# Borda/pyImSegm

Measured on NVIDIA H100. Metric: megapixels/sec end-to-end SLIC+features+GC (pipe_color2d_slic_features_model_graphcut), higher is better.
Workload: dtype f64

## Files before the change

### pyimsegm_b200/csrc/common.cuh

```cuda
#pragma once
#include <cuda_runtime.h>
#include <stdint.h>
#include <stdio.h>
#include "../../include/imsegm_b200.h"

void isb_set_error(const char* fmt, ...);
extern long long g_isb_launches;

enum {
    ISB_PROF_PREPARE = 0, ISB_PROF_ASSIGN, ISB_PROF_UPDATE, ISB_PROF_FINALIZE, ISB_PROF_CONN, ISB_PROF_STATS, ISB_PROF_ADJ,
    ISB_PROF_ENERGY, ISB_PROF_GC, ISB_PROF_GATHER, ISB_PROF_GMM, ISB_PROF_LM, ISB_PROF_COUNT
};
int isb_prof_begin(int id, cudaStream_t st);
void isb_prof_end(int handle, cudaStream_t st);
struct ProfScope {
    int h; cudaStream_t st;
    ProfScope(int id, cudaStream_t s) : h(isb_prof_begin(id, s)), st(s) {}
    ~ProfScope() { if (h >= 0) isb_prof_end(h, st); }
};

#define ISB_CUDA_CHECK(call)                                                                      \
    do {                                                                                          \
        cudaError_t e__ = (call);                                                                 \
        if (e__ != cudaSuccess) {                                                                 \
            isb_set_error("%s:%d %s -> %s", __FILE__, __LINE__, #call, cudaGetErrorString(e__));  \
            return ISB_ERR_CUDA;                                                                  \
        }                                                                                         \
    } while (0)

#define ISB_LAUNCH_CHECK()                                                                        \
    do {                                                                                          \
        ++g_isb_launches;                                                                         \
        cudaError_t e__ = cudaGetLastError();                                                     \
        if (e__ != cudaSuccess) {                                                                 \
            isb_set_error("%s:%d kernel launch -> %s", __FILE__, __LINE__, cudaGetErrorString(e__)); \
            return ISB_ERR_CUDA;                                                                  \
        }                                                                                         \
    } while (0)

#define ISB_REQUIRE(cond, msg)                                          \
    do {                                                                \
        if (!(cond)) {                                                  \
            isb_set_error("%s:%d %s", __FILE__, __LINE__, msg);         \
            return ISB_ERR_ARG;                                         \
        }                                                               \
    } while (0)

static inline size_t isb_align(size_t x, size_t a = 256) { return (x + a - 1) / a * a; }

struct WsCarver {
    char* base;
    size_t off, cap;
    WsCarver(void* p, size_t bytes) : base((char*)p), off(0), cap(bytes) {}
    template <typename T> T* take(size_t n)
    {
        size_t o = isb_align(off);
        off = o + n * sizeof(T);
        return (T*)(base + o);
    }
    bool ok() const { return off <= cap; }
};

__device__ __forceinline__ double load_as_f64(const void* p, int dtype, size_t i)
{
    switch (dtype) {
        case ISB_U8: return (double)((const unsigned char*)p)[i];
        case ISB_U16: return (double)((const unsigned short*)p)[i];
        case ISB_F32: return (double)((const float*)p)[i];
        default: return ((const double*)p)[i];
    }
}

__device__ __forceinline__ float load_as_f32(const void* p, int dtype, size_t i)
{
    switch (dtype) {
        case ISB_U8: return (float)((const unsigned char*)p)[i];
        case ISB_U16: return (float)((const unsigned short*)p)[i];
        case ISB_F32: return ((const float*)p)[i];
        default: return (float)((const double*)p)[i];
    }
}

__device__ __forceinline__ unsigned long long f64_ordered(double d)
{
    unsigned long long u = (unsigned long long)__double_as_longlong(d);
    return (u & 0x8000000000000000ull) ? ~u : (u | 0x8000000000000000ull);
}
__device__ __forceinline__ double f64_unordered(unsigned long long u)
{
    u = (u & 0x8000000000000000ull) ? (u & 0x7FFFFFFFFFFFFFFFull) : ~u;
    return __longlong_as_double((long long)u);
}

__device__ __forceinline__ int reflect_index(int i, int n)
{
    if ((unsigned)i < (unsigned)n) return i;
    if (n == 1) return 0;
    int p = 2 * n;
    i %= p;
    if (i < 0) i += p;
    return (i < n) ? i : (p - 1 - i);
}
```

### pyimsegm_b200/csrc/graph.cu

```cuda
#include "common.cuh"
#include "block_scan.cuh"
#include <cooperative_groups.h>
namespace cg = cooperative_groups;

namespace {


struct AdjWs {
    unsigned long long* table;
    int* ctr;
    int* deg;
    int* off;
    int* fill;
    int* tmp_a;
    int slots;
    size_t zeroed;
};

__device__ __forceinline__ unsigned hash64(unsigned long long k)
{
    k ^= k >> 33; k *= 0xff51afd7ed558ccdull; k ^= k >> 33; k *= 0xc4ceb9fe1a85ec53ull; k ^= k >> 33;
    return (unsigned)k;
}

__device__ __forceinline__ unsigned long long edge_key(int l0, int l1)
{
    return ((unsigned long long)(unsigned)max(l0, l1) << 32) | (unsigned)min(l0, l1);
}

__device__ void table_insert(const AdjWs& w, unsigned long long key)
{
    unsigned mask = (unsigned)w.slots - 1u;
    unsigned h = hash64(key) & mask;
    for (int probe = 0; probe < w.slots; ++probe) {
        unsigned long long cur = w.table[h];
        if (cur == key) return;
        if (cur == 0) {
            unsigned long long old = atomicCAS(&w.table[h], 0ull, key);
            if (old == 0) { atomicAdd(&w.deg[key >> 32], 1); atomicAdd(&w.ctr[0], 1); return; }
            if (old == key) return;
        }
        h = (h + 1) & mask;
    }
    atomicExch(&w.ctr[1], 1);
}

constexpr int CTA_SLOTS = 512, CTA_PROBES = 32;

__device__ void cta_set_clear(unsigned long long* s)
{
    for (int i = threadIdx.x; i < CTA_SLOTS; i += blockDim.x) s[i] = 0;
    __syncthreads();
}

__device__ void cta_set_insert(unsigned long long* s, const AdjWs& w, unsigned long long key)
{
    unsigned h = hash64(key) & (CTA_SLOTS - 1);
    for (int probe = 0; probe < CTA_PROBES; ++probe) {
        unsigned long long cur = s[h];
        if (cur == key) return;
        if (cur == 0) {
            cur = atomicCAS(&s[h], 0ull, key);
            if (cur == 0 || cur == key) return;
        }
        h = (h + 1) & (CTA_SLOTS - 1);
    }
    table_insert(w, key);
}

__device__ void cta_set_flush(const unsigned long long* s, const AdjWs& w)
{
    __syncthreads();
    for (int i = threadIdx.x; i < CTA_SLOTS; i += blockDim.x)
        if (s[i]) table_insert(w, s[i]);
}

constexpr int ETW = 64, ETR = 4, ETH = ETR * (256 / ETW);

__global__ void __launch_bounds__(256) k_edge_scan(const int* __restrict__ seg, int H, int W, AdjWs w)
{
    __shared__ unsigned long long s_set[CTA_SLOTS];
    cta_set_clear(s_set);
    const int x = blockIdx.x * ETW + (int)(threadIdx.x % ETW);
    const int y0 = blockIdx.y * ETH + (int)(threadIdx.x / ETW) * ETR, y1 = min(y0 + ETR, H);
    if (x < W && y0 < H) {
        unsigned long long last = 0;
        int l = seg[(size_t)y0 * W + x];
        for (int y = y0; y < y1; ++y) {
            const size_t p = (size_t)y * W + x;
            const int d = y + 1 < H ? seg[p + W] : l;
            if (x + 1 < W) {
                const int r = seg[p + 1];
                if (r != l && edge_key(l, r) != last) { last = edge_key(l, r); cta_set_insert(s_set, w, last); }
            }
            if (d != l && edge_key(l, d) != last) { last = edge_key(l, d); cta_set_insert(s_set, w, last); }
            l = d;
        }
    }
    cta_set_flush(s_set, w);
}

__global__ void __launch_bounds__(256) k_edge_scan3d(const int* __restrict__ seg, int D, int H, int W, AdjWs w)
{
    __shared__ unsigned long long s_set[CTA_SLOTS];
    cta_set_clear(s_set);
    const size_t p = (size_t)blockIdx.x * blockDim.x + threadIdx.x;
    if (p < (size_t)D * H * W) {
        const int x = (int)(p % W), y = (int)((p / W) % H), z = (int)(p / ((size_t)H * W));
        const int l = seg[p];
        if (x + 1 < W) { const int r = seg[p + 1]; if (r != l) cta_set_insert(s_set, w, edge_key(l, r)); }
        if (y + 1 < H) { const int d = seg[p + W]; if (d != l) cta_set_insert(s_set, w, edge_key(l, d)); }
        if (z + 1 < D) { const int b = seg[p + (size_t)H * W]; if (b != l) cta_set_insert(s_set, w, edge_key(l, b)); }
    }
    cta_set_flush(s_set, w);
}

__global__ void k_centroid3d_acc(const int* __restrict__ seg, int D, int H, int W, unsigned long long* acc)
{
    size_t p = (size_t)blockIdx.x * blockDim.x + threadIdx.x;
    if (p >= (size_t)D * H * W) return;
    const int x = (int)(p % W), y = (int)((p / W) % H), z = (int)(p / ((size_t)H * W));
    unsigned long long* a = acc + 4 * (size_t)seg[p];
    atomicAdd(a, 1ull); atomicAdd(a + 1, (unsigned long long)z); atomicAdd(a + 2, (unsigned long long)y); atomicAdd(a + 3, (unsigned long long)x);
}

__global__ void k_centroid3d_fin(int nb, const unsigned long long* acc, double* centres)
{
    const int k = blockIdx.x * blockDim.x + threadIdx.x;
    if (k >= nb) return;
    const double c = (double)acc[4 * (size_t)k];
    for (int d = 0; d < 3; ++d) centres[3 * (size_t)k + d] = c > 0 ? (double)acc[4 * (size_t)k + 1 + d] / c : -1.0;
}

__global__ void __launch_bounds__(1024) k_edge_offsets(int nb, AdjWs w, int cap, int* n_edges_out)
{
    const int total = cta_scan_chunks<1024, int>(nb, [&](int i) { return w.deg[i]; },
                                                 [&](int i, int off) { w.off[i] = off; w.fill[i] = 0; });
    if (threadIdx.x == 0) {
        w.off[nb] = total;
        *n_edges_out = (w.ctr[1] || total > cap) ? cap + 1 : total;
    }
}

__global__ void k_edge_fill(AdjWs w, int cap)
{
    int i = blockIdx.x * blockDim.x + threadIdx.x;
    if (i >= w.slots) return;
    unsigned long long key = w.table[i];
    if (key == 0) return;
    int b = (int)(key >> 32), a = (int)(key & 0xffffffffu);
    int pos = w.off[b] + atomicAdd(&w.fill[b], 1);
    if (pos < cap) w.tmp_a[pos] = a;
}

__global__ void k_edge_emit(int nb, AdjWs w, int cap, int* __restrict__ edges)
{
    int b = blockIdx.x * blockDim.x + threadIdx.x;
    if (b >= nb) return;
    int beg = w.off[b], end = w.off[b + 1];
    if (end > cap) return;
    for (int i = beg + 1; i < end; ++i) {
        int v = w.tmp_a[i], j = i - 1;
        while (j >= beg && w.tmp_a[j] > v) { w.tmp_a[j + 1] = w.tmp_a[j]; --j; }
        w.tmp_a[j + 1] = v;
    }
    for (int i = beg; i < end; ++i) { edges[2 * (size_t)i] = w.tmp_a[i]; edges[2 * (size_t)i + 1] = b; }
}

static int pow2_at_least(long long v) { int p = 1024; while (p < v) p <<= 1; return p; }

static size_t carve_adj(AdjWs& w, void* ws, size_t bytes, int nb, int cap)
{
    WsCarver c(ws, bytes);
    w.slots = pow2_at_least(2LL * cap);
    w.table = c.take<unsigned long long>((size_t)w.slots);
    w.ctr = c.take<int>(4);
    w.deg = c.take<int>(nb);
    w.zeroed = c.off;
    w.off = c.take<int>((size_t)nb + 1);
    w.fill = c.take<int>(nb);
    w.tmp_a = c.take<int>(cap);
    return isb_align(c.off);
}


__device__ double block_sum(double v, double* s_red)
{
#pragma unroll
    for (int o = 16; o > 0; o >>= 1) v += __shfl_xor_sync(0xffffffffu, v, o);
    __syncthreads();
    if ((threadIdx.x & 31) == 0) s_red[threadIdx.x >> 5] = v;
    __syncthreads();
    double t = 0;
    for (int i = 0; i < (int)(blockDim.x >> 5); ++i) t += s_red[i];
    return t;
}

__device__ double block_max(double v, double* s_red)
{
#pragma unroll
    for (int o = 16; o > 0; o >>= 1) v = fmax(v, __shfl_xor_sync(0xffffffffu, v, o));
    __syncthreads();
    if ((threadIdx.x & 31) == 0) s_red[threadIdx.x >> 5] = v;
    __syncthreads();
    double t = s_red[0];
    for (int i = 1; i < (int)(blockDim.x >> 5); ++i) t = fmax(t, s_red[i]);
    return t;
}

constexpr int ECL = 8;

__device__ double cluster_reduce(double v, bool is_max, double* s_red, double* s_x)
{
    const double t = is_max ? block_max(v, s_red) : block_sum(v, s_red);
    cg::cluster_group cl = cg::this_cluster();
    if (threadIdx.x == 0) *s_x = t;
    cl.sync();
    double tot = is_max ? -1.0 : 0.0;
    for (int r = 0; r < ECL; ++r) { const double pr = *cl.map_shared_rank(s_x, r); tot = is_max ? fmax(tot, pr) : tot + pr; }
    cl.sync();
    return tot;
}

__global__ void __cluster_dims__(ECL, 1, 1) __launch_bounds__(1024) k_gc_energies(const double* __restrict__ proba, int N_in, const int* n_nodes_dev, int K, const int* __restrict__ edges, int E_in,
                                                      const int* n_edges_dev, const double* __restrict__ centres,
                                                      const double* __restrict__ vfeat, int D, int metric, int spatial,
                                                      double edge_cost, const double* __restrict__ pairwise, double* unary,
                                                      double* edge_w, int* unary_i, int* edge_wi, int* smooth_i, double* sp)
{
    __shared__ double s_red[32];
    __shared__ double s_x;
    const int tid = blockIdx.x * blockDim.x + threadIdx.x, nth = gridDim.x * blockDim.x;
    const int E = n_edges_dev ? (*n_edges_dev > E_in ? 0 : *n_edges_dev) : E_in;
    const int N = n_nodes_dev ? min(*n_nodes_dev, N_in) : N_in;
    double umax = 0.0;
    for (int i = tid; i < N * K; i += nth) {
        double p = proba[i];
        if (p < 0.01) p = 0.01;
        if (p > 1.0 - 0.01) p = 1.0 - 0.01;
        double u = fabs(-log(p));
        unary[i] = u;
        umax = fmax(umax, fabs(u));
    }
    umax = cluster_reduce(umax, true, s_red, &s_x);
    double dsum = 0.0, ssum = 0.0;
    for (int e = tid; e < E; e += nth) {
        int a = edges[2 * e], b = edges[2 * e + 1];
        double dist = 0.0;
        if (metric != 0) {
            const double* va = vfeat + (size_t)a * D;
            const double* vb = vfeat + (size_t)b * D;
            for (int k = 0; k < D; ++k) {
                double df = va[k] - vb[k];
                if (metric == 1) dist = fmax(dist, df * df);
                else if (metric == 2) dist += fabs(df);
                else dist += df * df;
            }
            if (metric == 3) dist = sqrt(dist);
        }
        edge_w[e] = dist;
        dsum += dist;
        if (spatial == 3) {
            const double cz = centres[3 * a] - centres[3 * b], cy = centres[3 * a + 1] - centres[3 * b + 1];
            const double cx = centres[3 * a + 2] - centres[3 * b + 2];
            const double s = sqrt(cz * cz + cy * cy + cx * cx);
            sp[e] = s;
            ssum += s;
        } else if (spatial) {
            double cy = centres[2 * a] - centres[2 * b], cx = centres[2 * a + 1] - centres[2 * b + 1];
            double s = sqrt(cy * cy + cx * cx);
            sp[e] = s;
            ssum += s;
        }
    }
    dsum = cluster_reduce(dsum, false, s_red, &s_x);
    ssum = cluster_reduce(ssum, false, s_red, &s_x);
    const double dmean = E > 0 ? dsum / E : 0.0, smean = E > 0 ? ssum / E : 1.0;
    double vsum = 0.0;
    if (metric != 0)
        for (int e = tid; e < E; e += nth) { double t = edge_w[e] - dmean; vsum += t * t; }
    vsum = cluster_reduce(vsum, false, s_red, &s_x);
    const double sd = sqrt(E > 0 ? vsum / E : 0.0);
    const double denom = 2.0 * (sd * sd);
    double wmax = 0.0;
    for (int e = tid; e < E; e += nth) {
        double wv = metric != 0 ? exp(-edge_w[e] / denom) : 1.0;
        if (spatial) wv = wv / (sp[e] / smean);
        if (wv < 1e-3) wv = 1e-3;
        if (wv > 1e3) wv = 1e3;
        wv *= edge_cost;
        edge_w[e] = wv;
        wmax = fmax(wmax, fabs(wv));
    }
    wmax = cluster_reduce(wmax, true, s_red, &s_x);
    double pmax = pairwise[0];
    for (int i = 1; i < K * K; ++i) pmax = fmax(pmax, pairwise[i]);
    const double dwf = fmax(umax, wmax * pmax) + 1e-10;
    for (int i = tid; i < N * K; i += nth) unary_i[i] = (int)((unary[i] / dwf) * 100000.0);
    for (int e = tid; e < E; e += nth) { const double wv = edge_w[e]; edge_wi[e] = isnan(wv) ? 0 : (int)((wv / dwf) * 1000.0); }
    for (int i = tid; i < K * K; i += nth) smooth_i[i] = (int)(pairwise[i] * 100.0);
}


constexpr int GV = 4, GW = 32 * GV;

__global__ void __launch_bounds__(256) k_gather(const int* __restrict__ seg, long long n, long long n_vec, const int* __restrict__ lut_i,
                                                const double* __restrict__ lut_p, int K, int* __restrict__ out_i, double* __restrict__ out_p)
{
    __shared__ int s_lab[256 * GV];
    const long long p0 = ((long long)blockIdx.x * blockDim.x + threadIdx.x) * GV;
    if (p0 >= n) return;
    if (p0 < n_vec) {
        const int4 l = *reinterpret_cast<const int4*>(seg + p0);
        if (out_i) *reinterpret_cast<int4*>(out_i + p0) = make_int4(__ldg(lut_i + l.x), __ldg(lut_i + l.y), __ldg(lut_i + l.z), __ldg(lut_i + l.w));
        if (out_p) {
            const int lane = threadIdx.x & 31;
            *reinterpret_cast<int4*>(s_lab + threadIdx.x * GV) = l;
            __syncwarp();
            const int* lab = s_lab + (threadIdx.x - lane) * GV;
            double2* dst = reinterpret_cast<double2*>(out_p + (p0 - lane * GV) * K);
            int q = 2 * lane / K, k = 2 * lane % K;
            const int dq = 64 / K, dk = 64 % K;
#pragma unroll 2
            for (int i = lane; i < GW * K / 2; i += 32) {
                const double v0 = __ldg(lut_p + (size_t)lab[q] * K + k);
                const int q1 = k + 1 == K ? q + 1 : q, k1 = k + 1 == K ? 0 : k + 1;
                const double v1 = __ldg(lut_p + (size_t)lab[q1] * K + k1);
                dst[i] = make_double2(v0, v1);
                q += dq; k += dk;
                if (k >= K) { k -= K; ++q; }
            }
        }
        return;
    }
    for (long long p = p0; p < min(p0 + GV, n); ++p) {
        const int l = seg[p];
        if (out_i) out_i[p] = lut_i[l];
        if (out_p) {
            const double* src = lut_p + (size_t)l * K;
            double* dst = out_p + (size_t)p * K;
            for (int k = 0; k < K; ++k) dst[k] = src[k];
        }
    }
}

}

extern "C" size_t isb_adjacency_workspace_bytes(int nb, int cap)
{
    AdjWs w;
    return carve_adj(w, nullptr, 0, nb, cap);
}

extern "C" int isb_adjacency_edges(const int32_t* seg, int H, int W, int nb, int32_t* edges, int cap, int32_t* n_edges_out, void* ws,
                                   size_t ws_bytes, isb_stream_t stream)
{
    ISB_REQUIRE(seg && edges && n_edges_out && ws, "null pointer");
    ISB_REQUIRE(H > 0 && W > 0 && nb > 0 && cap > 0, "bad sizes");
    ISB_REQUIRE((H + ETH - 1) / ETH <= 65535, "label map taller than the scan grid (1 048 560 rows)");
    AdjWs w;
    size_t need = carve_adj(w, ws, ws_bytes, nb, cap);
    ISB_REQUIRE(need <= ws_bytes, "workspace too small");
    cudaStream_t st = (cudaStream_t)stream;
    ProfScope prof(ISB_PROF_ADJ, st);
    ISB_CUDA_CHECK(cudaMemsetAsync(w.table, 0, w.zeroed, st));
    k_edge_scan<<<dim3((W + ETW - 1) / ETW, (H + ETH - 1) / ETH), 256, 0, st>>>(seg, H, W, w);
    ISB_LAUNCH_CHECK();
    k_edge_offsets<<<1, 1024, 0, st>>>(nb, w, cap, n_edges_out);
    ISB_LAUNCH_CHECK();
    k_edge_fill<<<(w.slots + 255) / 256, 256, 0, st>>>(w, cap);
    ISB_LAUNCH_CHECK();
    k_edge_emit<<<(nb + 127) / 128, 128, 0, st>>>(nb, w, cap, edges);
    ISB_LAUNCH_CHECK();
    return ISB_OK;
}

extern "C" int isb_adjacency_edges_3d(const int32_t* seg, int D, int H, int W, int nb, int32_t* edges, int cap, int32_t* n_edges_out,
                                      void* ws, size_t ws_bytes, isb_stream_t stream)
{
    ISB_REQUIRE(seg && edges && n_edges_out && ws, "null pointer");
    ISB_REQUIRE(D > 0 && H > 0 && W > 0 && nb > 0 && cap > 0, "bad sizes");
    AdjWs w;
    size_t need = carve_adj(w, ws, ws_bytes, nb, cap);
    ISB_REQUIRE(need <= ws_bytes, "workspace too small");
    cudaStream_t st = (cudaStream_t)stream;
    ProfScope prof(ISB_PROF_ADJ, st);
    ISB_CUDA_CHECK(cudaMemsetAsync(w.table, 0, w.zeroed, st));
    size_t n = (size_t)D * H * W;
    k_edge_scan3d<<<(unsigned)((n + 255) / 256), 256, 0, st>>>(seg, D, H, W, w);
    ISB_LAUNCH_CHECK();
    k_edge_offsets<<<1, 1024, 0, st>>>(nb, w, cap, n_edges_out);
    ISB_LAUNCH_CHECK();
    k_edge_fill<<<(w.slots + 255) / 256, 256, 0, st>>>(w, cap);
    ISB_LAUNCH_CHECK();
    k_edge_emit<<<(nb + 127) / 128, 128, 0, st>>>(nb, w, cap, edges);
    ISB_LAUNCH_CHECK();
    return ISB_OK;
}

extern "C" int isb_centroids_3d(const int32_t* seg, int D, int H, int W, int nb, double* centres, void* ws, size_t ws_bytes, isb_stream_t stream)
{
    ISB_REQUIRE(seg && centres && ws, "null pointer");
    ISB_REQUIRE(D > 0 && H > 0 && W > 0 && nb > 0, "bad sizes");
    ISB_REQUIRE(ws_bytes >= sizeof(unsigned long long) * 4 * (size_t)nb, "workspace too small (4 * nb uint64)");
    cudaStream_t st = (cudaStream_t)stream;
    ISB_CUDA_CHECK(cudaMemsetAsync(ws, 0, sizeof(unsigned long long) * 4 * (size_t)nb, st));
    size_t n = (size_t)D * H * W;
    k_centroid3d_acc<<<(unsigned)((n + 255) / 256), 256, 0, st>>>(seg, D, H, W, (unsigned long long*)ws);
    ISB_LAUNCH_CHECK();
    k_centroid3d_fin<<<(nb + 255) / 256, 256, 0, st>>>(nb, (const unsigned long long*)ws, centres);
    ISB_LAUNCH_CHECK();
    return ISB_OK;
}

extern "C" size_t isb_gc_energies_workspace_bytes(int N, int K, int E) { return isb_align(sizeof(double) * (size_t)(E > 0 ? E : 1)); }

extern "C" int isb_gc_energies(const double* proba, int N, const int32_t* n_nodes_dev, int K, const int32_t* edges, int E, const int32_t* n_edges_dev,
                               const double* centres, int metric, int spatial, double edge_cost, const double* pairwise, double* unary,
                               double* edge_w, int32_t* unary_i, int32_t* edge_wi, int32_t* smooth_i, void* ws, size_t ws_bytes,
                               isb_stream_t stream)
{
    ISB_REQUIRE(proba && edges && pairwise && unary && edge_w && unary_i && edge_wi && smooth_i && ws, "null pointer");
    ISB_REQUIRE(N > 0 && K > 0 && E >= 0, "bad sizes");
    ISB_REQUIRE(metric >= 0 && metric <= 3, "metric must be 0..3");
    ISB_REQUIRE(spatial >= 0 && spatial <= 3, "spatial must be 0 (off), 1 or 2 (centres [N, 2]) or 3 (centres [N, 3])");
    ISB_REQUIRE(!spatial || centres, "centres are required for spatially normalised edge weights");
    ISB_REQUIRE(ws_bytes >= isb_gc_energies_workspace_bytes(N, K, E), "workspace too small");
    ProfScope prof(ISB_PROF_ENERGY, (cudaStream_t)stream);
    k_gc_energies<<<ECL, 1024, 0, (cudaStream_t)stream>>>(proba, N, n_nodes_dev, K, edges, E, n_edges_dev, centres, proba, K, metric, spatial, edge_cost,
                                                         pairwise, unary, edge_w, unary_i, edge_wi, smooth_i, (double*)ws);
    ISB_LAUNCH_CHECK();
    return ISB_OK;
}

__global__ void k_fill_i32(int* p, long long n, int v)
{
    long long i = (long long)blockIdx.x * blockDim.x + threadIdx.x;
    if (i < n) p[i] = v;
}

extern "C" int isb_fill_i32(int32_t* dst, long long n, int32_t value, isb_stream_t stream)
{
    ISB_REQUIRE(dst && n > 0, "bad arguments");
    k_fill_i32<<<(unsigned)((n + 255) / 256), 256, 0, (cudaStream_t)stream>>>(dst, n, value);
    ISB_LAUNCH_CHECK();
    return ISB_OK;
}

__global__ void k_combine(void* dst, const void* src, long long n, int op)
{
    long long i = (long long)blockIdx.x * blockDim.x + threadIdx.x;
    if (i >= n) return;
    if (op == 0) ((long long*)dst)[i] += ((const long long*)src)[i];
    else if (op == 1) { long long a = ((long long*)dst)[i], b = ((const long long*)src)[i]; ((long long*)dst)[i] = a > b ? a : b; }
    else if (op == 2 || op == 3) {
        const double a = ((double*)dst)[i], b = ((const double*)src)[i];
        ((double*)dst)[i] = (a != a || b != b) ? a + b : (op == 2 ? fmin(a, b) : fmax(a, b));
    }
    else ((double*)dst)[i] = ((double*)dst)[i] + ((const double*)src)[i];
}

extern "C" int isb_combine(void* dst, const void* src, long long n, int op, isb_stream_t stream)
{
    ISB_REQUIRE(dst && src && n > 0 && op >= 0 && op <= 4, "bad arguments");
    k_combine<<<(unsigned)((n + 255) / 256), 256, 0, (cudaStream_t)stream>>>(dst, src, n, op);
    ISB_LAUNCH_CHECK();
    return ISB_OK;
}

extern "C" int isb_gather(const int32_t* seg, long long npx, const int32_t* lut_i, const double* lut_p, int K, int32_t* out_i,
                          double* out_p, isb_stream_t stream)
{
    ISB_REQUIRE(seg && npx > 0, "bad arguments");
    ISB_REQUIRE((!out_i || lut_i) && (!out_p || (lut_p && K > 0)), "LUT missing for a requested output");
    ProfScope prof(ISB_PROF_GATHER, (cudaStream_t)stream);
    const bool aligned = (((uintptr_t)seg | (uintptr_t)out_i | (uintptr_t)out_p) & 15) == 0;
    const long long groups = (npx + GV - 1) / GV;
    k_gather<<<(unsigned)((groups + 255) / 256), 256, 0, (cudaStream_t)stream>>>(seg, npx, aligned ? npx / GW * GW : 0, lut_i, lut_p, K,
                                                                                out_i, out_p);
    ISB_LAUNCH_CHECK();
    return ISB_OK;
}
```

### pyimsegm_b200/csrc/slic_connectivity.cu

```cuda
#include "common.cuh"
#include "block_scan.cuh"

namespace {

constexpr int TH = 32, TW = 64, TPIX = TH * TW;
constexpr int WIN = 4096;
constexpr int RANK_WORDS = 1024;

enum { C_OVER = 0, C_FALLBACK = 1, C_QUEUE = 2, C_LROOTS = 3, C_WINDOW = 4, C_N = 8 };

struct ConnWs {
    int* parent;
    int* size;
    int* ymax;
    int* xmin;
    int* xmax;
    int* aux;
    int* lroots;
    int* window;
    int* fallback;
    int* over;
    int* ctr;
    int* blk;
    unsigned* kept;
};

constexpr int VISBIT = 1 << 30;
__device__ __forceinline__ int dec(int c) { return (c < 0 ? ~c : c) & ~VISBIT; }

__device__ __forceinline__ int resolve(const int* parent, int p)
{
    const int a = parent[p];
    return dec(a < 0 ? a : parent[a & ~VISBIT]);
}

__device__ __forceinline__ int find_root(const int* parent, int i)
{
    while (true) {
        int p = parent[i];
        if (p == i) return i;
        i = p;
    }
}

__device__ __forceinline__ void unite(int* parent, int a, int b)
{
    while (true) {
        a = find_root(parent, a);
        b = find_root(parent, b);
        if (a == b) return;
        if (a < b) { int t = a; a = b; b = t; }
        int old = atomicMin(&parent[a], b);
        if (old == a) return;
        a = old;
    }
}

__device__ __forceinline__ int sfind(const volatile int* par, int i)
{
    while (true) {
        int p = par[i];
        if (p == i) return i;
        i = p;
    }
}

__device__ __forceinline__ void sunite(int* par, int a, int b)
{
    while (true) {
        a = sfind(par, a);
        b = sfind(par, b);
        if (a == b) return;
        if (a < b) { int t = a; a = b; b = t; }
        int old = atomicMin(&par[a], b);
        if (old == a) return;
        a = old;
    }
}

__device__ __forceinline__ void mark_kept(int r, unsigned* kept, int* blk)
{
    atomicOr(&kept[r >> 5], 1u << (r & 31));
    atomicAdd(&blk[r / (32 * RANK_WORDS)], 1);
}

__global__ void __launch_bounds__(256, 5) k_ccl_tile(const int* __restrict__ lab, int H, int W, int ntx, int* __restrict__ parent,
                                                  int* __restrict__ size, int* __restrict__ ymax, int* __restrict__ xmin,
                                                  int* __restrict__ xmax, int* __restrict__ lroots, int* ctr)
{
    constexpr int PT = TPIX / 256;
    __shared__ int s_lab[TPIX];
    __shared__ int s_par[TPIX];
    __shared__ int s_ymax[TPIX], s_xmin[TPIX], s_xmax[TPIX];
    __shared__ unsigned s_starts[TPIX / 32];
    const int x0 = (blockIdx.x % ntx) * TW, y0 = (blockIdx.x / ntx) * TH;
    const int tw = min(TW, W - x0), th = min(TH, H - y0);
    const int lane = threadIdx.x & 31;
#pragma unroll
    for (int k = 0; k < PT; ++k) {
        const int i = threadIdx.x + 256 * k, ly = i / TW, lx = i % TW;
        s_lab[i] = (ly < th && lx < tw) ? lab[(size_t)(y0 + ly) * W + x0 + lx] : 0;
        s_ymax[i] = -1; s_xmin[i] = INT_MAX; s_xmax[i] = -1;
    }
    __syncthreads();
#pragma unroll
    for (int k = 0; k < PT; ++k) {
        const int i = threadIdx.x + 256 * k, ly = i / TW, lx = i % TW;
        const bool start = lx == 0 || lx >= tw || ly >= th || s_lab[i - 1] != s_lab[i];
        const unsigned m = __ballot_sync(0xffffffffu, start);
        if (lane == 0) s_starts[i / 32] = m;
    }
    __syncthreads();
#pragma unroll
    for (int k = 0; k < PT; ++k) {
        const int i = threadIdx.x + 256 * k, ly = i / TW, lx = i % TW;
        const unsigned long long row = ((unsigned long long)s_starts[2 * ly + 1] << 32) | s_starts[2 * ly];
        s_par[i] = ly * TW + 63 - __clzll(row & (~0ull >> (63 - lx)));
    }
    __syncthreads();
#pragma unroll
    for (int k = 0; k < PT; ++k) {
        const int i = threadIdx.x + 256 * k, ly = i / TW, lx = i % TW;
        if (ly == 0 || ly >= th || lx >= tw) continue;
        const int l = s_lab[i];
        if (s_lab[i - TW] != l) continue;
        if (lx > 0 && s_lab[i - 1] == l && s_lab[i - TW - 1] == l) continue;
        sunite(s_par, i, i - TW);
    }
    __syncthreads();
#pragma unroll
    for (int k = 0; k < PT; ++k) {
        const int i = threadIdx.x + 256 * k;
        if ((s_starts[i / 32] >> (i % 32)) & 1u) s_par[i] = sfind(s_par, i);
    }
    __syncthreads();
#pragma unroll
    for (int k = 0; k < PT; ++k) {
        const int i = threadIdx.x + 256 * k;
        if (!((s_starts[i / 32] >> (i % 32)) & 1u)) s_par[i] = s_par[s_par[i]];
        s_lab[i] = 0;
    }
    __syncthreads();
#pragma unroll
    for (int k = 0; k < PT; ++k) {
        const int i = threadIdx.x + 256 * k, ly = i / TW, lx = i % TW;
        if (ly >= th || lx >= tw || !((s_starts[i / 32] >> (i % 32)) & 1u)) continue;
        const unsigned long long row = ((unsigned long long)s_starts[2 * ly + 1] << 32) | s_starts[2 * ly];
        const unsigned long long rest = lx == TW - 1 ? 0ull : row >> (lx + 1);
        const int len = rest ? __ffsll((long long)rest) : TW - lx;
        const int r = s_par[i];
        atomicAdd(&s_lab[r], len);
        atomicMax(&s_ymax[r], ly);
        atomicMin(&s_xmin[r], lx);
        atomicMax(&s_xmax[r], lx + len - 1);
    }
    __syncthreads();
#pragma unroll
    for (int k = 0; k < PT; ++k) {
        const int i = threadIdx.x + 256 * k, ly = i / TW, lx = i % TW;
        const bool valid = ly < th && lx < tw;
        const int p = (y0 + ly) * W + x0 + lx;
        const int r = s_par[i];
        const bool is_root = valid && r == i;
        if (valid) parent[p] = (y0 + r / TW) * W + x0 + r % TW;
        if (is_root) {
            size[p] = s_lab[i];
            ymax[p] = y0 + s_ymax[i]; xmin[p] = x0 + s_xmin[i]; xmax[p] = x0 + s_xmax[i];
        }
        const unsigned m = __ballot_sync(0xffffffffu, is_root);
        int base = 0;
        if (lane == 0 && m) base = atomicAdd(&ctr[C_LROOTS], __popc(m));
        base = __shfl_sync(0xffffffffu, base, 0);
        if (is_root) lroots[base + __popc(m & ((1u << lane) - 1u))] = p;
    }
}

__global__ void k_ccl_seams(const int* __restrict__ lab, int H, int W, int nvs, int nhs, int* parent)
{
    int t = blockIdx.x * blockDim.x + threadIdx.x;
    if (t >= nvs + nhs) return;
    int p, q;
    if (t < nvs) {
        const int k = t / H, y = t - k * H, x = (k + 1) * TW;
        p = y * W + x; q = p - 1;
        const int l = lab[p];
        if (lab[q] != l) return;
        if (y % TH != 0 && lab[p - W] == l && lab[q - W] == l) return;
    } else {
        t -= nvs;
        const int k = t / W, x = t - k * W, y = (k + 1) * TH;
        p = y * W + x; q = p - W;
        const int l = lab[p];
        if (lab[q] != l) return;
        if (x % TW != 0 && lab[p - 1] == l && lab[q - 1] == l) return;
    }
    unite(parent, p, q);
}

__global__ void k_ccl_roots(int* parent, int* size, int* ymax, int* xmin, int* xmax, const int* __restrict__ lroots,
                            const int* __restrict__ ctr)
{
    const int n = ctr[C_LROOTS];
    for (int i = blockIdx.x * blockDim.x + threadIdx.x; i < n; i += gridDim.x * blockDim.x) {
        const int lr = lroots[i];
        const int g = find_root(parent, lr);
        if (g == lr) continue;
        parent[lr] = g;
        atomicAdd(&size[g], size[lr]);
        atomicMax(&ymax[g], ymax[lr]);
        atomicMin(&xmin[g], xmin[lr]);
        atomicMax(&xmax[g], xmax[lr]);
    }
}

__global__ void k_ccl_classify(int H, int W, int min_size, int max_size, const int* __restrict__ parent, const int* __restrict__ size,
                               const int* __restrict__ ymax, const int* __restrict__ xmin, const int* __restrict__ xmax,
                               const int* __restrict__ lroots, int* ctr, int* over, int* window, int* fallback, unsigned* kept, int* blk)
{
    const int n = ctr[C_LROOTS];
    for (int i = blockIdx.x * blockDim.x + threadIdx.x; i < n; i += gridDim.x * blockDim.x) {
        const int g = lroots[i];
        if (parent[g] != g) continue;
        const int s = size[g];
        if (s >= max_size) {
            over[atomicAdd(&ctr[C_OVER], 1)] = g;
        } else if (s >= min_size) {
            mark_kept(g, kept, blk);
        } else {
            const int y = g / W;
            const int wh = min(ymax[g] + 1, H - 1) - max(y - 1, 0) + 1;
            const int ww = min(xmax[g] + 1, W - 1) - max(xmin[g] - 1, 0) + 1;
            if (wh * ww <= WIN) window[atomicAdd(&ctr[C_WINDOW], 1)] = g;
            else fallback[atomicAdd(&ctr[C_FALLBACK], 1)] = g;
        }
    }
}

__global__ void k_ccl_flatten(int n, int* parent, const int* __restrict__ ctr)
{
    if (ctr[C_OVER] == 0 && ctr[C_FALLBACK] == 0) return;
    for (int p = blockIdx.x * blockDim.x + threadIdx.x; p < n; p += gridDim.x * blockDim.x) parent[p] = parent[parent[p]];
}

__global__ void k_oversize_split(int H, int W, int* comp, int* size, const int* __restrict__ ymax, const int* __restrict__ xmin,
                                 const int* __restrict__ xmax, int min_size, int max_size, const int* __restrict__ list, int* ctr,
                                 int* fallback, unsigned* kept, int* blk, int* queue)
{
    int i = blockIdx.x * blockDim.x + threadIdx.x;
    if (i >= ctr[C_OVER]) return;
    const int C = list[i];
    const int4 bb = make_int4(C / W, ymax[C], xmin[C], xmax[C]);
    int* q = queue + (size_t)i * max_size;
    const int total = size[C];
    int assigned = 0;
    for (int y = bb.x; y <= bb.y && assigned < total; ++y)
        for (int x = bb.z; x <= bb.w && assigned < total; ++x) {
            int p = y * W + x;
            if (comp[p] != C) continue;
            int start = p;
            comp[p] = ~start;
            q[0] = p;
            int n = 1, v = 0;
            while (v < n && n < max_size) {
                int cp = q[v];
                int cy = cp / W, cx = cp - cy * W;
                const int nx[4] = { cx + 1, cx - 1, cx, cx };
                const int ny[4] = { cy, cy, cy + 1, cy - 1 };
                for (int d = 0; d < 4; ++d) {
                    if (nx[d] < 0 || nx[d] >= W || ny[d] < 0 || ny[d] >= H) continue;
                    int np_ = ny[d] * W + nx[d];
                    if (comp[np_] == C) {
                        comp[np_] = ~start;
                        q[n++] = np_;
                        if (n >= max_size) break;
                    }
                }
                ++v;
            }
            size[start] = n;
            assigned += n;
            if (n >= min_size) mark_kept(start, kept, blk);
            else fallback[atomicAdd(&ctr[C_FALLBACK], 1)] = start;
        }
}

__global__ void __launch_bounds__(256) k_kept_ranks(int n_words, const unsigned* __restrict__ kept, const int* __restrict__ blk,
                                                    int* aux, int* n_labels_out)
{
    constexpr int WPT = RANK_WORDS / 256;
    int part = 0;
    for (int j = threadIdx.x; j < (int)blockIdx.x; j += 256) part += blk[j];
    unsigned bits[WPT];
    int c = 0;
#pragma unroll
    for (int k = 0; k < WPT; ++k) {
        const int w = blockIdx.x * RANK_WORDS + threadIdx.x * WPT + k;
        bits[k] = w < n_words ? kept[w] : 0u;
        c += __popc(bits[k]);
    }
    int base, tot;
    cta_exclusive_sum<256>(part, base);
    int label = base + cta_exclusive_sum<256>(c, tot);
#pragma unroll
    for (int k = 0; k < WPT; ++k) {
        const int w = blockIdx.x * RANK_WORDS + threadIdx.x * WPT + k;
        for (unsigned b = bits[k]; b; b &= b - 1) aux[w * 32 + __ffs(b) - 1] = label++;
    }
    if (blockIdx.x == gridDim.x - 1 && threadIdx.x == 0) *n_labels_out = base + tot > 0 ? base + tot : 1;
}

__global__ void __launch_bounds__(256) k_small_window(int H, int W, const int* __restrict__ parent, const int* __restrict__ ymax,
                                                      const int* __restrict__ xmin, const int* __restrict__ xmax,
                                                      const int* __restrict__ list, const int* __restrict__ ctr, int* __restrict__ aux)
{
    __shared__ int s_id[WIN];
    __shared__ int s_q[WIN];
    const int n_small = ctr[C_WINDOW];
    for (int i = blockIdx.x; i < n_small; i += gridDim.x) {
        const int C = list[i];
        const int y = C / W, x = C - y * W;
        const int wy0 = max(y - 1, 0), wx0 = max(xmin[C] - 1, 0);
        const int wh = min(ymax[C] + 1, H - 1) - wy0 + 1, ww = min(xmax[C] + 1, W - 1) - wx0 + 1;
        const int area = wh * ww;
#pragma unroll 4
        for (int j = threadIdx.x; j < area; j += 256) {
            const int jy = j / ww;
            s_id[j] = resolve(parent, (wy0 + jy) * W + wx0 + j - jy * ww);
        }
        __syncthreads();
        if (threadIdx.x == 0) {
            int adjacent = -1;
            const int cy0 = y - wy0, cx0 = x - wx0;
            s_q[0] = (cy0 << 16) | cx0;
            s_id[cy0 * ww + cx0] = INT_MAX;
            int n = 1;
            for (int v = 0; v < n; ++v) {
                const int cy = s_q[v] >> 16, cx = s_q[v] & 0xffff;
                const int c = cy * ww + cx, gy = wy0 + cy, gx = wx0 + cx;
                const bool ok4[4] = { gx + 1 < W, gx > 0, gy + 1 < H, gy > 0 };
                const int nc4[4] = { c + 1, c - 1, c + ww, c - ww };
                const int nq4[4] = { (cy << 16) | (cx + 1), (cy << 16) | (cx - 1), ((cy + 1) << 16) | cx, ((cy - 1) << 16) | cx };
                int r4[4];
#pragma unroll
                for (int d = 0; d < 4; ++d) r4[d] = ok4[d] ? s_id[nc4[d]] : INT_MAX;
#pragma unroll
                for (int d = 0; d < 4; ++d) {
                    if (r4[d] == C) {
                        s_id[nc4[d]] = INT_MAX;
                        s_q[n++] = nq4[d];
                    } else if (r4[d] < C) {
                        adjacent = r4[d];
                    }
                }
            }
            aux[C] = adjacent >= 0 ? -2 - adjacent : -1;
        }
        __syncthreads();
    }
}

template <bool SQ>
__global__ void __launch_bounds__(SQ ? 32 : 256) k_small_adjacent(int H, int W, int* comp, const int* __restrict__ size, int max_size,
                                                                   const int* __restrict__ list, int* ctr, int* aux, int* queue)
{
    extern __shared__ int s_q[];
    const int n_small = ctr[1];
    for (int i = blockIdx.x * blockDim.x + threadIdx.x; i < n_small; i += gridDim.x * blockDim.x) {
        const int C = list[i];
        int* q = SQ ? s_q + threadIdx.x : queue + atomicAdd(&ctr[2], size[C]);
        constexpr int QS = SQ ? 32 : 1;
        int adjacent = -1;
        q[0] = C;
        comp[C] = (comp[C] < 0 ? ~(dec(comp[C]) | VISBIT) : (comp[C] | VISBIT));
        int n = 1, v = 0;
        while (v < n && n < max_size) {
            const int cp = q[v * QS];
            const int cy = cp / W, cx = cp - cy * W;
            const int np4[4] = { cx + 1 < W ? cp + 1 : -1, cx > 0 ? cp - 1 : -1, cy + 1 < H ? cp + W : -1, cy > 0 ? cp - W : -1 };
            int raw4[4];
#pragma unroll
            for (int d = 0; d < 4; ++d) raw4[d] = np4[d] >= 0 ? comp[np4[d]] : 0;
#pragma unroll
            for (int d = 0; d < 4; ++d) {
                if (np4[d] < 0) continue;
                const int raw = raw4[d];
                const int r = dec(raw);
                if (r == C) {
                    const bool seen = ((raw < 0 ? ~raw : raw) & VISBIT) != 0;
                    if (!seen) {
                        comp[np4[d]] = raw < 0 ? ~((~raw) | VISBIT) : (raw | VISBIT);
                        q[(n++) * QS] = np4[d];
                        if (n >= max_size) break;
                    }
                } else if (r < C) {
                    adjacent = r;
                }
            }
            ++v;
        }
        aux[C] = adjacent >= 0 ? -2 - adjacent : -1;
    }
}

constexpr int WRITE_PX = 4;
__global__ void __launch_bounds__(256) k_ccl_write(int n, const int* __restrict__ parent, const int* __restrict__ aux,
                                                   int* __restrict__ out)
{
    const int p0 = blockIdx.x * 256 * WRITE_PX + threadIdx.x;
    int r[WRITE_PX], a[WRITE_PX];
#pragma unroll
    for (int k = 0; k < WRITE_PX; ++k) r[k] = p0 + 256 * k < n ? parent[p0 + 256 * k] : 0;
#pragma unroll
    for (int k = 0; k < WRITE_PX; ++k) r[k] = dec(r[k] < 0 ? r[k] : parent[r[k] & ~VISBIT]);
#pragma unroll
    for (int k = 0; k < WRITE_PX; ++k) a[k] = aux[r[k]];
#pragma unroll
    for (int k = 0; k < WRITE_PX; ++k) {
        while (a[k] < -1) { r[k] = -2 - a[k]; a[k] = aux[r[k]]; }
        if (p0 + 256 * k < n) out[p0 + 256 * k] = a[k] < 0 ? 0 : a[k];
    }
}

static size_t carve(ConnWs& w, void* ws, size_t bytes, int H, int W, int* n_zero)
{
    WsCarver c(ws, bytes);
    size_t n = (size_t)H * W;
    w.parent = c.take<int>(n); w.size = c.take<int>(n);
    w.ymax = c.take<int>(n); w.xmin = c.take<int>(n); w.xmax = c.take<int>(n);
    w.aux = c.take<int>(n); w.lroots = c.take<int>(n); w.window = c.take<int>(n); w.fallback = c.take<int>(n);
    w.over = c.take<int>(n / 16 + 16);
    const size_t n_words = (n + 31) / 32, n_blk = (n_words + RANK_WORDS - 1) / RANK_WORDS;
    w.ctr = c.take<int>(C_N + n_blk + n_words);
    w.blk = w.ctr + C_N;
    w.kept = (unsigned*)(w.blk + n_blk);
    *n_zero = (int)(C_N + n_blk + n_words);
    return isb_align(c.off);
}

}

extern "C" size_t isb_connectivity_workspace_bytes(int H, int W)
{
    ConnWs w;
    int n_zero;
    return carve(w, nullptr, 0, H, W, &n_zero);
}

extern "C" int isb_enforce_connectivity(const int32_t* labels, int H, int W, int min_size, int max_size, int32_t* out,
                                        int32_t* n_labels_out, void* ws, size_t ws_bytes, isb_stream_t stream)
{
    ISB_REQUIRE(labels && out && n_labels_out && ws, "null pointer");
    ISB_REQUIRE(H > 0 && W > 0 && (long long)H * W < (1LL << 30), "bad image size (at most 2^30 pixels)");
    if (max_size < 1) max_size = 1;
    ISB_REQUIRE(max_size >= 16, "max_size < 16 is not supported on the device path (oversize table bound)");
    ConnWs w;
    int n_zero;
    size_t need = carve(w, ws, ws_bytes, H, W, &n_zero);
    ISB_REQUIRE(need <= ws_bytes, "workspace too small");
    cudaStream_t st = (cudaStream_t)stream;
    ProfScope prof(ISB_PROF_CONN, st);
    const int n = H * W;
    const int ntx = (W + TW - 1) / TW, nty = (H + TH - 1) / TH;
    const int n_words = (n + 31) / 32, n_rank = (n_words + RANK_WORDS - 1) / RANK_WORDS;
    int dev = 0, sms = 0;
    ISB_CUDA_CHECK(cudaGetDevice(&dev));
    ISB_CUDA_CHECK(cudaDeviceGetAttribute(&sms, cudaDevAttrMultiProcessorCount, dev));
    ISB_CUDA_CHECK(cudaMemsetAsync(w.ctr, 0, sizeof(int) * (size_t)n_zero, st));
    k_ccl_tile<<<ntx * nty, 256, 0, st>>>(labels, H, W, ntx, w.parent, w.size, w.ymax, w.xmin, w.xmax, w.lroots, w.ctr);
    ISB_LAUNCH_CHECK();
    const int nvs = (ntx - 1) * H, nhs = (nty - 1) * W;
    if (nvs + nhs > 0) {
        k_ccl_seams<<<(nvs + nhs + 255) / 256, 256, 0, st>>>(labels, H, W, nvs, nhs, w.parent);
        ISB_LAUNCH_CHECK();
    }
    k_ccl_roots<<<sms * 4, 256, 0, st>>>(w.parent, w.size, w.ymax, w.xmin, w.xmax, w.lroots, w.ctr);
    ISB_LAUNCH_CHECK();
    k_ccl_classify<<<sms * 4, 256, 0, st>>>(H, W, min_size, max_size, w.parent, w.size, w.ymax, w.xmin, w.xmax, w.lroots, w.ctr,
                                            w.over, w.window, w.fallback, w.kept, w.blk);
    ISB_LAUNCH_CHECK();
    k_ccl_flatten<<<sms * 8, 256, 0, st>>>(n, w.parent, w.ctr);
    ISB_LAUNCH_CHECK();
    const int n_over_max = n / max_size + 1;
    k_oversize_split<<<(n_over_max + 63) / 64, 64, 0, st>>>(H, W, w.parent, w.size, w.ymax, w.xmin, w.xmax, min_size, max_size, w.over,
                                                            w.ctr, w.fallback, w.kept, w.blk, w.lroots);
    ISB_LAUNCH_CHECK();
    k_kept_ranks<<<n_rank, 256, 0, st>>>(n_words, w.kept, w.blk, w.aux, n_labels_out);
    ISB_LAUNCH_CHECK();
    k_small_window<<<sms * 6, 256, 0, st>>>(H, W, w.parent, w.ymax, w.xmin, w.xmax, w.window, w.ctr, w.aux);
    ISB_LAUNCH_CHECK();
    if (min_size >= 1 && min_size <= 512) {
        const size_t smem = sizeof(int) * 32 * (size_t)min_size;
        ISB_CUDA_CHECK(cudaFuncSetAttribute(k_small_adjacent<true>, cudaFuncAttributeMaxDynamicSharedMemorySize, (int)smem));
        k_small_adjacent<true><<<sms * 16, 32, smem, st>>>(H, W, w.parent, w.size, max_size, w.fallback, w.ctr, w.aux, w.lroots);
    } else {
        k_small_adjacent<false><<<sms * 8, 256, 0, st>>>(H, W, w.parent, w.size, max_size, w.fallback, w.ctr, w.aux, w.lroots);
    }
    ISB_LAUNCH_CHECK();
    k_ccl_write<<<(n + 256 * WRITE_PX - 1) / (256 * WRITE_PX), 256, 0, st>>>(n, w.parent, w.aux, out);
    ISB_LAUNCH_CHECK();
    return ISB_OK;
}
```

Before: 1618.

## Restructure edge scan, offsets scan, and CCL root compaction; add phase stamps

The edge scan now processes 8 rows per thread. It preloads each column strip into registers and gets right-neighbour labels with warp shuffles instead of extra global loads. The global edge counter atomic is dropped. The offsets kernel uses a blocked shared-memory scan with padding to avoid bank conflicts, and CCL tile labelling uses path-halving finds plus one per-CTA root compaction with a single atomic. Optional globaltimer phase stamps are added behind a compile flag for profiling; the dropped counter could matter if anything still reads ctr[0].

After: 1627 (median of 6 runs). Within noise of the previous version (+0.6%).

```diff
diff --git a/pyimsegm_b200/csrc/common.cuh b/pyimsegm_b200/csrc/common.cuh
--- a/pyimsegm_b200/csrc/common.cuh
+++ b/pyimsegm_b200/csrc/common.cuh
@@ -45,6 +45,22 @@
             return ISB_ERR_ARG;                                         \
         }                                                               \
     } while (0)
+
+#ifdef ISB_PHASE_STAMPS
+constexpr int ISB_STAMP_CTAS = 8192, ISB_STAMP_SLOTS = 8;
+#define ISB_STAMP(buf, k)                                                                         \
+    do {                                                                                          \
+        __syncthreads();                                                                          \
+        const unsigned cta__ = blockIdx.y * gridDim.x + blockIdx.x;                               \
+        if (threadIdx.x == 0 && cta__ < (unsigned)ISB_STAMP_CTAS) {                               \
+            unsigned long long t__;                                                               \
+            asm volatile("mov.u64 %0, %%globaltimer;" : "=l"(t__));                              \
+            (buf)[cta__ * ISB_STAMP_SLOTS + (k)] = t__;                                           \
+        }                                                                                         \
+    } while (0)
+#else
+#define ISB_STAMP(buf, k) do { } while (0)
+#endif
 
 static inline size_t isb_align(size_t x, size_t a = 256) { return (x + a - 1) / a * a; }
 
diff --git a/pyimsegm_b200/csrc/graph.cu b/pyimsegm_b200/csrc/graph.cu
--- a/pyimsegm_b200/csrc/graph.cu
+++ b/pyimsegm_b200/csrc/graph.cu
@@ -37,7 +37,7 @@
         if (cur == key) return;
         if (cur == 0) {
             unsigned long long old = atomicCAS(&w.table[h], 0ull, key);
-            if (old == 0) { atomicAdd(&w.deg[key >> 32], 1); atomicAdd(&w.ctr[0], 1); return; }
+            if (old == 0) { atomicAdd(&w.deg[key >> 32], 1); return; }
             if (old == key) return;
         }
         h = (h + 1) & mask;
@@ -75,29 +75,44 @@
         if (s[i]) table_insert(w, s[i]);
 }
 
-constexpr int ETW = 64, ETR = 4, ETH = ETR * (256 / ETW);
+constexpr int ETW = 64, ETR = 8, ETH = ETR * (256 / ETW);
+
+#ifdef ISB_PHASE_STAMPS
+__device__ unsigned long long g_stamps_edge[ISB_STAMP_CTAS * ISB_STAMP_SLOTS];
+#endif
 
 __global__ void __launch_bounds__(256) k_edge_scan(const int* __restrict__ seg, int H, int W, AdjWs w)
 {
     __shared__ unsigned long long s_set[CTA_SLOTS];
+    ISB_STAMP(g_stamps_edge, 0);
+    const int lane = threadIdx.x & 31;
+    const int x = blockIdx.x * ETW + (int)(threadIdx.x % ETW);
+    const int y0 = blockIdx.y * ETH + (int)(threadIdx.x / ETW) * ETR;
+    int c[ETR + 1], r[ETR];
+#pragma unroll
+    for (int k = 0; k <= ETR; ++k) c[k] = x < W && y0 + k < H ? seg[(size_t)(y0 + k) * W + x] : 0;
+#pragma unroll
+    for (int k = 0; k < ETR; ++k) r[k] = lane == 31 && x + 1 < W && y0 + k < H ? seg[(size_t)(y0 + k) * W + x + 1] : 0;
+#pragma unroll
+    for (int k = 0; k < ETR; ++k) {
+        const int n = __shfl_down_sync(0xffffffffu, c[k], 1);
+        if (lane != 31) r[k] = n;
+    }
     cta_set_clear(s_set);
-    const int x = blockIdx.x * ETW + (int)(threadIdx.x % ETW);
-    const int y0 = blockIdx.y * ETH + (int)(threadIdx.x / ETW) * ETR, y1 = min(y0 + ETR, H);
-    if (x < W && y0 < H) {
+    ISB_STAMP(g_stamps_edge, 1);
+    if (x < W) {
         unsigned long long last = 0;
-        int l = seg[(size_t)y0 * W + x];
-        for (int y = y0; y < y1; ++y) {
-            const size_t p = (size_t)y * W + x;
-            const int d = y + 1 < H ? seg[p + W] : l;
-            if (x + 1 < W) {
-                const int r = seg[p + 1];
-                if (r != l && edge_key(l, r) != last) { last = edge_key(l, r); cta_set_insert(s_set, w, last); }
-            }
+#pragma unroll
+        for (int k = 0; k < ETR; ++k) {
+            if (y0 + k >= H) break;
+            const int l = c[k], d = y0 + k + 1 < H ? c[k + 1] : l;
+            if (x + 1 < W && r[k] != l && edge_key(l, r[k]) != last) { last = edge_key(l, r[k]); cta_set_insert(s_set, w, last); }
             if (d != l && edge_key(l, d) != last) { last = edge_key(l, d); cta_set_insert(s_set, w, last); }
-            l = d;
-        }
-    }
+        }
+    }
+    ISB_STAMP(g_stamps_edge, 2);
     cta_set_flush(s_set, w);
+    ISB_STAMP(g_stamps_edge, 3);
 }
 
 __global__ void __launch_bounds__(256) k_edge_scan3d(const int* __restrict__ seg, int D, int H, int W, AdjWs w)
@@ -132,10 +147,36 @@
     for (int d = 0; d < 3; ++d) centres[3 * (size_t)k + d] = c > 0 ? (double)acc[4 * (size_t)k + 1 + d] / c : -1.0;
 }
 
+constexpr int OFF_IT = 8;
+__device__ __forceinline__ int off_slot(int j) { return j + j / 32; }
+
 __global__ void __launch_bounds__(1024) k_edge_offsets(int nb, AdjWs w, int cap, int* n_edges_out)
 {
-    const int total = cta_scan_chunks<1024, int>(nb, [&](int i) { return w.deg[i]; },
-                                                 [&](int i, int off) { w.off[i] = off; w.fill[i] = 0; });
+    __shared__ int s_d[1024 * OFF_IT + 1024 * OFF_IT / 32];
+    int total = 0;
+    for (int base = 0; base < nb; base += 1024 * OFF_IT) {
+        int d[OFF_IT];
+#pragma unroll
+        for (int k = 0; k < OFF_IT; ++k) d[k] = base + k * 1024 + (int)threadIdx.x < nb ? w.deg[base + k * 1024 + threadIdx.x] : 0;
+#pragma unroll
+        for (int k = 0; k < OFF_IT; ++k) s_d[off_slot(k * 1024 + threadIdx.x)] = d[k];
+        __syncthreads();
+        int sum = 0;
+#pragma unroll
+        for (int k = 0; k < OFF_IT; ++k) { d[k] = s_d[off_slot(threadIdx.x * OFF_IT + k)]; sum += d[k]; }
+        int round;
+        int off = total + cta_exclusive_sum<1024>(sum, round);
+#pragma unroll
+        for (int k = 0; k < OFF_IT; ++k) { s_d[off_slot(threadIdx.x * OFF_IT + k)] = off; off += d[k]; }
+        __syncthreads();
+#pragma unroll
+        for (int k = 0; k < OFF_IT; ++k) {
+            const int i = base + k * 1024 + threadIdx.x;
+            if (i < nb) { w.off[i] = s_d[off_slot(k * 1024 + threadIdx.x)]; w.fill[i] = 0; }
+        }
+        __syncthreads();
+        total += round;
+    }
     if (threadIdx.x == 0) {
         w.off[nb] = total;
         *n_edges_out = (w.ctr[1] || total > cap) ? cap + 1 : total;
@@ -346,6 +387,13 @@
 
 }
 
+#ifdef ISB_PHASE_STAMPS
+extern "C" int isb_debug_stamps_edge(unsigned long long* host)
+{
+    return cudaMemcpyFromSymbol(host, g_stamps_edge, sizeof(g_stamps_edge)) == cudaSuccess ? ISB_OK : ISB_ERR_CUDA;
+}
+#endif
+
 extern "C" size_t isb_adjacency_workspace_bytes(int nb, int cap)
 {
     AdjWs w;
@@ -357,7 +405,7 @@
 {
     ISB_REQUIRE(seg && edges && n_edges_out && ws, "null pointer");
     ISB_REQUIRE(H > 0 && W > 0 && nb > 0 && cap > 0, "bad sizes");
-    ISB_REQUIRE((H + ETH - 1) / ETH <= 65535, "label map taller than the scan grid (1 048 560 rows)");
+    ISB_REQUIRE((H + ETH - 1) / ETH <= 65535, "label map taller than the scan grid (2 097 120 rows)");
     AdjWs w;
     size_t need = carve_adj(w, ws, ws_bytes, nb, cap);
     ISB_REQUIRE(need <= ws_bytes, "workspace too small");
diff --git a/pyimsegm_b200/csrc/slic_connectivity.cu b/pyimsegm_b200/csrc/slic_connectivity.cu
--- a/pyimsegm_b200/csrc/slic_connectivity.cu
+++ b/pyimsegm_b200/csrc/slic_connectivity.cu
@@ -6,6 +6,10 @@
 constexpr int TH = 32, TW = 64, TPIX = TH * TW;
 constexpr int WIN = 4096;
 constexpr int RANK_WORDS = 1024;
+
+#ifdef ISB_PHASE_STAMPS
+__device__ unsigned long long g_stamps_ccl[ISB_STAMP_CTAS * ISB_STAMP_SLOTS];
+#endif
 
 enum { C_OVER = 0, C_FALLBACK = 1, C_QUEUE = 2, C_LROOTS = 3, C_WINDOW = 4, C_N = 8 };
 
@@ -65,11 +69,23 @@
     }
 }
 
+__device__ __forceinline__ int sfind_halving(volatile int* par, int i)
+{
+    while (true) {
+        const int p = par[i];
+        if (p == i) return i;
+        const int g = par[p];
+        if (g == p) return p;
+        par[i] = g;
+        i = g;
+    }
+}
+
 __device__ __forceinline__ void sunite(int* par, int a, int b)
 {
     while (true) {
-        a = sfind(par, a);
-        b = sfind(par, b);
+        a = sfind_halving(par, a);
+        b = sfind_halving(par, b);
         if (a == b) return;
         if (a < b) { int t = a; a = b; b = t; }
         int old = atomicMin(&par[a], b);
@@ -93,9 +109,12 @@
     __shared__ int s_par[TPIX];
     __shared__ int s_ymax[TPIX], s_xmin[TPIX], s_xmax[TPIX];
     __shared__ unsigned s_starts[TPIX / 32];
+    __shared__ unsigned s_roots[TPIX / 32];
+    __shared__ int s_rbase[TPIX / 32];
     const int x0 = (blockIdx.x % ntx) * TW, y0 = (blockIdx.x / ntx) * TH;
     const int tw = min(TW, W - x0), th = min(TH, H - y0);
     const int lane = threadIdx.x & 31;
+    ISB_STAMP(g_stamps_ccl, 0);
 #pragma unroll
     for (int k = 0; k < PT; ++k) {
         const int i = threadIdx.x + 256 * k, ly = i / TW, lx = i % TW;
@@ -103,6 +122,7 @@
         s_ymax[i] = -1; s_xmin[i] = INT_MAX; s_xmax[i] = -1;
     }
     __syncthreads();
+    ISB_STAMP(g_stamps_ccl, 1);
 #pragma unroll
     for (int k = 0; k < PT; ++k) {
         const int i = threadIdx.x + 256 * k, ly = i / TW, lx = i % TW;
@@ -118,6 +138,7 @@
         s_par[i] = ly * TW + 63 - __clzll(row & (~0ull >> (63 - lx)));
     }
     __syncthreads();
+    ISB_STAMP(g_stamps_ccl, 2);
 #pragma unroll
     for (int k = 0; k < PT; ++k) {
         const int i = threadIdx.x + 256 * k, ly = i / TW, lx = i % TW;
@@ -128,6 +149,7 @@
         sunite(s_par, i, i - TW);
     }
     __syncthreads();
+    ISB_STAMP(g_stamps_ccl, 3);
 #pragma unroll
     for (int k = 0; k < PT; ++k) {
         const int i = threadIdx.x + 256 * k;
@@ -136,11 +158,28 @@
     __syncthreads();
 #pragma unroll
     for (int k = 0; k < PT; ++k) {
-        const int i = threadIdx.x + 256 * k;
+        const int i = threadIdx.x + 256 * k, ly = i / TW, lx = i % TW;
         if (!((s_starts[i / 32] >> (i % 32)) & 1u)) s_par[i] = s_par[s_par[i]];
         s_lab[i] = 0;
-    }
-    __syncthreads();
+        const unsigned m = __ballot_sync(0xffffffffu, ly < th && lx < tw && s_par[i] == i);
+        if (lane == 0) s_roots[i / 32] = m;
+    }
+    __syncthreads();
+    ISB_STAMP(g_stamps_ccl, 4);
+    if (threadIdx.x < 32) {
+        const int c0 = __popc(s_roots[2 * lane]), c = c0 + __popc(s_roots[2 * lane + 1]);
+        int incl = c;
+#pragma unroll
+        for (int o = 1; o < 32; o <<= 1) {
+            const int t = __shfl_up_sync(0xffffffffu, incl, o);
+            if (lane >= o) incl += t;
+        }
+        int base = 0;
+        if (lane == 31 && incl) base = atomicAdd(&ctr[C_LROOTS], incl);
+        base = __shfl_sync(0xffffffffu, base, 31) + incl - c;
+        s_rbase[2 * lane] = base;
+        s_rbase[2 * lane + 1] = base + c0;
+    }
 #pragma unroll
     for (int k = 0; k < PT; ++k) {
         const int i = threadIdx.x + 256 * k, ly = i / TW, lx = i % TW;
@@ -155,6 +194,7 @@
         atomicMax(&s_xmax[r], lx + len - 1);
     }
     __syncthreads();
+    ISB_STAMP(g_stamps_ccl, 5);
 #pragma unroll
     for (int k = 0; k < PT; ++k) {
         const int i = threadIdx.x + 256 * k, ly = i / TW, lx = i % TW;
@@ -167,12 +207,9 @@
             size[p] = s_lab[i];
             ymax[p] = y0 + s_ymax[i]; xmin[p] = x0 + s_xmin[i]; xmax[p] = x0 + s_xmax[i];
         }
-        const unsigned m = __ballot_sync(0xffffffffu, is_root);
-        int base = 0;
-        if (lane == 0 && m) base = atomicAdd(&ctr[C_LROOTS], __popc(m));
-        base = __shfl_sync(0xffffffffu, base, 0);
-        if (is_root) lroots[base + __popc(m & ((1u << lane) - 1u))] = p;
-    }
+        if (is_root) lroots[s_rbase[i / 32] + __popc(s_roots[i / 32] & ((1u << lane) - 1u))] = p;
+    }
+    ISB_STAMP(g_stamps_ccl, 6);
 }
 
 __global__ void k_ccl_seams(const int* __restrict__ lab, int H, int W, int nvs, int nhs, int* parent)
@@ -439,6 +476,13 @@
 
 }
 
+#ifdef ISB_PHASE_STAMPS
+extern "C" int isb_debug_stamps_ccl(unsigned long long* host)
+{
+    return cudaMemcpyFromSymbol(host, g_stamps_ccl, sizeof(g_stamps_ccl)) == cudaSuccess ? ISB_OK : ISB_ERR_CUDA;
+}
+#endif
+
 extern "C" size_t isb_connectivity_workspace_bytes(int H, int W)
 {
     ConnWs w;
```
